# geopti/mjlab-1

Hardware: AMD Instinct MI355X
Metric: env-steps/sec, Unitree-G1 velocity task num_envs=4096, 1/2/4/8 MI355X (higher is better)
Workload: dtype f32

## Files before the change

### mjlab-1_amd/csrc/capi.cpp

```cpp
#include <dlfcn.h>
#include <hip/hip_runtime.h>

#include <cmath>
#include <cstdio>
#include <cstring>
#include <map>
#include <memory>
#include <string>
#include <algorithm>
#include <vector>

#include "../../include/mjx355.h"
#include "engine.h"
#include "model_tables.h"

extern "C" {
typedef struct { int32_t device_type; int32_t device_id; } DLDevice;
typedef struct { uint8_t code; uint8_t bits; uint16_t lanes; } DLDataType;
typedef struct {
  void* data;
  DLDevice device;
  int32_t ndim;
  DLDataType dtype;
  int64_t* shape;
// ... 232 lines not shown
#define X_FLT(name, cnt, w)                                                              \
  {                                                                                      \
    const size_t n_ = (size_t)(cnt) * (w);                                               \
    std::vector<float> h_(desc->name, desc->name + n_);                                  \
    if (upload(m.get(), h_, dm.name)) return -1;                                         \
    dm.name##_ws = 0;                                                                    \
    m->host_float[#name] = std::move(h_);                                                \
    m->float_dims[#name] = {(int64_t)(cnt), (int64_t)(w)};                               \
  }
  MJX_MODEL_INT_FIELDS(X_INT)
  MJX_MODEL_FLOAT_FIELDS(X_FLT)
#undef X_INT
#undef X_FLT
  if (upload(m.get(), std::vector<uint64_t>(desc->dof_bodymask, desc->dof_bodymask + d.nv), dm.dof_bodymask))
    return -1;
  dm.nmaskword = t.nmaskword;
  dm.neq = t.neq;
  dm.max_condim = t.max_condim;
  dm.ncsens = t.ncsens;
  const size_t nmask = (size_t)desc->nmaskword * d.nsensor;
  if (upload(m.get(), t.dof_ancmask, dm.dof_ancmask) || upload(m.get(), t.body_submask, dm.body_submask) ||
      upload(m.get(), t.body_dofmask, dm.body_dofmask) ||
      upload(m.get(), t.body_rec, dm.body_rec, mjx::kBodyRec) ||
      upload(m.get(), t.dof_rec, dm.dof_rec, mjx::kDofRec) ||
      upload(m.get(), t.act_rec, dm.act_rec, mjx::kActRec) ||
      upload(m.get(), t.geom_lds, dm.geom_lds) || upload(m.get(), t.lds_geom, dm.lds_geom) ||
      upload(m.get(), t.st_geom, dm.st_geom) || upload(m.get(), t.st_pairadr, dm.st_pairadr) ||
      upload(m.get(), t.st_partner, dm.st_partner) || upload(m.get(), t.st_aabb, dm.st_aabb, 6) ||
      upload(m.get(), t.st_chunk_aabb, dm.st_chunk_aabb) ||
      (!t.pair_rec.empty() && upload(m.get(), t.pair_rec, dm.pair_rec)) ||
      upload(m.get(), std::vector<uint32_t>(desc->sensor_geommask1, desc->sensor_geommask1 + nmask), dm.sensor_geommask1) ||
      upload(m.get(), std::vector<uint32_t>(desc->sensor_geommask2, desc->sensor_geommask2 + nmask), dm.sensor_geommask2) ||
      upload(m.get(), t.cs_sensor, dm.cs_sensor) || upload(m.get(), t.geom_csmask1, dm.geom_csmask1) ||
      upload(m.get(), t.geom_csmask2, dm.geom_csmask2))
    return -1;
  if (!t.sensor_ext.empty() && upload(m.get(), t.sensor_ext, m->ext.rec)) return -1;
  m->ext.n = (int)t.sensor_ext.size();
  *out = m.release();
  return 0;
}

int mjx_model_destroy(mjxModel* m) {
  if (m) delete m;
  return 0;
}

int mjx_sim_create(const mjxModel* model, int nworld, int nconmax, int njmax, mjxSim** out) {
  return mjx_sim_create_ex(model, nworld, nconmax, njmax, nconmax, njmax, out);
}

int mjx_sim_create_ex(const mjxModel* model, int nworld, int nconmax, int njmax,
                      int nconmax_max, int njmax_max, mjxSim** out) {
  if (!model || !out) return fail("null argument");
  if (nworld <= 0) return fail("nworld must be positive");
  if (nconmax <= 0 || nconmax > mjx::kWave)
    return fail("nconmax (contacts held per world) must be in [1, 64]");
  if (njmax <= 0) return fail("njmax must be positive");
  if (njmax < 2 * model->t.neq)
    return fail("njmax below the model's equality rows (two per equality constraint)");
  if (model->t.max_condim > 3 && njmax_max < 2 * model->t.neq + 2 * (model->t.max_condim - 1))
    return fail("njmax_max below one contact of the model's largest condim (2 (condim - 1) rows "
                "behind the equality rows)");
  if (nconmax_max < nconmax || nconmax_max > mjx::kMaxContacts || njmax_max < njmax)
    return fail("max capacity: nconmax <= nconmax_max <= 512 and njmax <= njmax_max");
  if (nconmax_max > mjx::kWave && nconmax_max > njmax_max)
    return fail("a max capacity past 64 contacts needs njmax_max >= nconmax_max (the contact sort's "
                "scratch is the row block)");
// ... 572 lines not shown
```

### mjlab-1_amd/csrc/engine.h

```cpp
#pragma once

#include <hip/hip_runtime.h>
#include <stddef.h>
#include <stdint.h>

#include "fields.h"

namespace mjx {

constexpr int kWave = 64;
constexpr int kMaxConRounds = 8;
constexpr int kMaxContacts = kWave * kMaxConRounds;
constexpr int kBodyRec = 20, kDofRec = 12, kActRec = 4;
constexpr int kMaxBodies = 64;
constexpr int kMaxDof = 64;
constexpr int kMaxLanes = 64;
constexpr int kRowClasses = 2;
constexpr int kMaxSplit = 4;
constexpr int kSplitMinWorlds = 2048;
constexpr int kMaxAirSlots = 8;
constexpr int kStaticChunk = 64;

enum { EFC_LIMIT = 0, EFC_FRICTIONLESS = 1, EFC_PYRAMIDAL = 2, EFC_EQUALITY = 3 };
constexpr int kMaxEq = 64;
enum { GEOM_PLANE = 0, GEOM_HFIELD = 1, GEOM_SPHERE = 2, GEOM_CAPSULE = 3, GEOM_BOX = 6 };
enum { JNT_FREE = 0, JNT_BALL = 1, JNT_SLIDE = 2, JNT_HINGE = 3 };
enum { SENS_GYRO = 0, SENS_VELOCIMETER = 1, SENS_ACCELEROMETER = 2, SENS_SUBTREEANGMOM = 3,
       SENS_CONTACT = 4, SENS_FRAMEPOS = 5, SENS_FRAMEQUAT = 6, SENS_JOINTPOS = 7,
       SENS_JOINTVEL = 8,
       SENS_FRAMEPOSX = 9, SENS_FRAMEXAXIS = 10, SENS_FRAMEYAXIS = 11, SENS_FRAMEZAXIS = 12,
       SENS_FRAMELINVEL = 13, SENS_FRAMEANGVEL = 14, SENS_FRAMELINACC = 15, SENS_FRAMEANGACC = 16,
       SENS_SUBTREECOM = 17, SENS_SUBTREELINVEL = 18, SENS_ACTUATORPOS = 19, SENS_ACTUATORVEL = 20,
       SENS_ACTUATORFRC = 21, SENS_JOINTACTUATORFRC = 22, SENS_COUNT = 23 };
enum { OBJ_NONE = 0, OBJ_BODY = 1, OBJ_XBODY = 2, OBJ_JOINT = 3, OBJ_GEOM = 5, OBJ_SITE = 6,
       OBJ_ACTUATOR = 19 };
enum { REDUCE_NONE = 0, REDUCE_MINDIST = 1, REDUCE_MAXFORCE = 2, REDUCE_NETFORCE = 3 };

struct Dims {
  int nq, nv, nu, nbody, njnt, ngeom, nsite, nsensor, nsensordata, npair;
  int nhfield, nhfielddata, nlevel, nchild, nmocap;
  int ngeom_lds;
  int npair_all;
  int nstatic;
  int nstpartner;
  int nboxbox;
  int nconmax;
// ... 12 lines not shown
#define X_FLT(name, cnt, w) const float* name; int name##_ws;
  MJX_MODEL_CORE_INT_FIELDS(X_INT)
  MJX_MODEL_CORE_FLOAT_FIELDS(X_FLT)
  const uint64_t* dof_bodymask;
  const uint64_t* dof_ancmask;
  const uint64_t* body_submask;
  const uint64_t* body_dofmask;
  const int32_t* body_rec;
  const int32_t* dof_rec;
  const int32_t* act_rec;
  const int32_t* geom_lds;
  const int32_t* lds_geom;
  const int32_t* st_geom;
  const int32_t* st_pairadr;
  const int32_t* st_partner;
  const float* st_aabb;
  const float* st_chunk_aabb;
  const int32_t* pair_rec;
  int nmaskword;
  const uint32_t* sensor_geommask1;
  const uint32_t* sensor_geommask2;
  int ncsens;
  const int32_t* cs_sensor;
  const uint64_t* geom_csmask1;
  const uint64_t* geom_csmask2;
  MJX_MODEL_EQ_INT_FIELDS(X_INT)
  MJX_MODEL_EQ_FLOAT_FIELDS(X_FLT)
#undef X_INT
#undef X_FLT
  int neq;
  int max_condim;
  int eq_reserved0;
  float* contact_torque;
  int eq_reserved[8];
};
static_assert(sizeof(DModel) - offsetof(DModel, eq_type) == 128, "DModel: the equality block is 128 bytes");

struct DData {
#define X_FLT(name, cnt, w) float* name;
#define X_INT(name, cnt, w) int32_t* name;
  MJX_DATA_FLOAT_FIELDS(X_FLT)
  MJX_DATA_INT_FIELDS(X_INT)
#undef X_FLT
#undef X_INT
  int32_t* stats;
  int32_t* wstats;
  int32_t* evtotal;
  unsigned long long* prof;
  unsigned long long* wtrace;
};

struct Lds {
  int qpos, qvel, ctrl, qacc_ws, qfrc_applied, xfrc;
  int xpos, xquat, xmat, xipos, ximat, xanchor, xaxis;
  int stmass, subtree_com, cinert, crb, cvel, cacc, stlin, stang;
  int cdof, cdofdot, cacc_v, gxpos, gxmat, sxpos, sxmat;
  int M, H;
  int qfrc_bias, qfrc_passive, qfrc_act, qfrc_smooth, qacc_smooth, x, Mx, grad, srch, Ms,
      qfrc_con, vtmp, act_force, act_len, act_vel;
  int con_g1, con_g2, con_key, con_dist, con_pos, con_frame, con_mu, con_kb,
      con_imp, con_imargin, con_dim, con_efc, con_n;
  int efc_J, efc_aref, efc_D, efc_jar, efc_Js, efc_force, efc_cid, efc_act, hdiag;
  int red;
  int chol;
  int ints;
  int pack_len;
  int packC_b;
// ... 169 lines not shown
```

### mjlab-1_amd/csrc/engine_impl.h

```cpp
#pragma once
#include <float.h>
#include <stdlib.h>
#include <algorithm>
#include <initializer_list>
#include <utility>
#include <math.h>

#include "engine.h"

#pragma clang fp contract(on)

namespace mjx {

#define MINVAL 1e-15f
#define MINMU 1e-5f
#define MINIMP 0.0001f
#define MAXIMP 0.9999f


struct V3 { float x, y, z; };
__device__ __forceinline__ V3 v3(const float* p) { return {p[0], p[1], p[2]}; }
__device__ __forceinline__ void st3(float* p, V3 a) { p[0] = a.x; p[1] = a.y; p[2] = a.z; }
__device__ __forceinline__ V3 operator+(V3 a, V3 b) { return {a.x + b.x, a.y + b.y, a.z + b.z}; }
__device__ __forceinline__ V3 operator-(V3 a, V3 b) { return {a.x - b.x, a.y - b.y, a.z - b.z}; }
// ... 506 lines not shown
#pragma unroll
  for (int c = 0; c < NR; c += 4) {
    float4 v = make_float4(0.f, 0.f, 0.f, 0.f);
    if (c < nvp) v = ld4(rp + c);
    A[c] = v.x; A[c + 1] = v.y; A[c + 2] = v.z; A[c + 3] = v.w;
  }
}
template <int NR>
__device__ __forceinline__ void rows_load_factor_ltr(float (&A)[NR], float& rd, const float* Lp,
                                                     int nvp, int lane) {
  const int ln = opaque_lane(lane);
  const int row = ln < nvp ? ln : 0;
  const float* rp = Lp + ltr_off(row);
  rows_load_ltr_span<NR>(A, rp, nvp);
  const float dv = rp[row];
  rd = ln < nvp ? dv : 1.f;
  const float ljj = __builtin_amdgcn_rcpf(rd);
#pragma unroll
  for (int k = 0; k < NR; k++) {
    const float s = rl(rd, k);
    A[k] = k < ln ? A[k] * (s * ljj) : 0.f;
  }
}
template <int NR>
__device__ __forceinline__ void rows_load_factor_ltr_raw(float (&A)[NR], float& dv, const float* Lp,
                                                         int nvp, int lane) {
  const int ln = opaque_lane(lane);
  const int row = ln < nvp ? ln : 0;
  const float* rp = Lp + ltr_off(row);
  const int len = 4 * ((row >> 2) + 1);
#pragma unroll
  for (int c = 0; c < NR; c += 4) {
    const float4 v = ld4(rp + (c < len ? c : 0));
    const bool in = c < len;
    A[c] = in ? v.x : 0.f; A[c + 1] = in ? v.y : 0.f; A[c + 2] = in ? v.z : 0.f; A[c + 3] = in ? v.w : 0.f;
  }
  dv = rp[row];
}
template <int NR>
__device__ __forceinline__ void rows_load_ltr(float (&A)[NR], const float* Lp, int nvp, int lane) {
  rows_load_ltr_span<NR>(A, Lp + ltr_off(lane < nvp ? lane : 0), nvp);
  if (NR > nvp || kWave > NR) {
    const int ln = opaque_lane(lane);
    const bool pad = ln >= nvp;
#pragma unroll
    for (int c = 0; c < NR; c++) A[c] = pad ? (c == ln ? 1.f : 0.f) : A[c];
  }
}
template <int NR>
__device__ __forceinline__ void rows_scale_factor_ltr(float (&A)[NR], float& rd, float dv, int nvp,
                                                      int lane) {
  const int ln = opaque_lane(lane);
  rd = ln < nvp ? dv : 1.f;
  const float ljj = __builtin_amdgcn_rcpf(rd);
#pragma unroll
  for (int k = 0; k < NR; k++) {
    const float s = rl(rd, k);
    A[k] = k < ln ? A[k] * (s * ljj) : 0.f;
  }
}
template <int NR>
__device__ __forceinline__ float rows_solve_ltr(const float (&M)[NR], float rdiag, const float* Lp,
                                                float x, int nvp, int lane) {
  float u = x;
#pragma unroll
  for (int j = 0; j < NR; j++) u = fmaf(-M[j], rl(u, j), u);
  float Nc[NR];
  const int ln = opaque_lane(lane);
  const int col = ln < nvp ? ln : 0;
#pragma unroll
// ... 1014 lines not shown
  unsigned long long z = seed + 0x9E3779B97F4A7C15ull * ((unsigned long long)(unsigned)w + 1) +
                         0xD1B54A32D192ED03ull * (unsigned long long)(unsigned)draw +
                         0x8CB92BA72F3D8DD7ull * (unsigned long long)group;
  z = (z ^ (z >> 30)) * 0xBF58476D1CE4E5B9ull;
  z = (z ^ (z >> 27)) * 0x94D049BB133111EBull;
  return (uint32_t)((z ^ (z >> 31)) >> 32);
}
__device__ __forceinline__ void act_push(const ActParams& A, int w, int u, int nu) {
  if (u >= nu || A.kind[u] == kActBuiltin || A.max_lag[u] == 0) return;
  const int L = A.ring_len;
  const size_t i = (size_t)w * nu + u;
  float* r = A.ring + (size_t)w * L * nu + u;
  for (int k = 0; k + 1 < L; k++) r[(size_t)k * nu] = r[(size_t)(k + 1) * nu];
  r[(size_t)(L - 1) * nu] = A.pt[i];
  A.pushes[i] = min(A.pushes[i] + 1, L);
  const int lo = A.min_lag[u], span = A.max_lag[u] - lo + 1;
  if (span > 1 && !(A.hold && A.hold[i])) {
    const int n = A.draws[i];
    A.lag[i] = lo + (int)(((unsigned long long)act_hash(A.seed, w, A.group[u], n) * (unsigned)span) >> 32);
    A.draws[i] = (int)((unsigned)n + 1u);
  }
}
__device__ __forceinline__ int cb_b1(int v) { return v & 255; }
__device__ __forceinline__ int cb_b2(int v) { return (v >> 8) & 255; }
__device__ __forceinline__ int cb_r1(int v) { return (v >> 16) & 255; }
__device__ __forceinline__ int cb_r2(int v) { return (v >> 24) & 255; }
__device__ __forceinline__ V3 point_vel_r(const float* S, const Lds& L, int b, int root, V3 p) {
  if (b <= 0) return {0.f, 0.f, 0.f};
  const float* cv = S + L.cvel + 6 * b;
  return v3(cv + 3) + cross(v3(cv), p - v3(S + L.subtree_com + 3 * root));
}

__device__ __forceinline__ void contact_sensors_wave(const float* S, const int* Si, const Lds& L,
                                                     const DModel& m, const Dims& d, float* sd,
                                                     int ncon, int maxmatch, bool all,
                                                     const Params* __restrict__ P, int lane,
                                                     int mcd, int cone) {
  const int c = lane;
  const bool valid = c < ncon;
  V3 fg = {0, 0, 0}, fc = {0, 0, 0}, tc = {0, 0, 0};
  float dist = 0.f;
  uint64_t m1 = 0, m2 = 0;
  if (valid) {
    const int g1 = Si[L.con_g1 + c], g2 = Si[L.con_g2 + c];
    m1 = m.geom_csmask1[g1] & m.geom_csmask2[g2];
    m2 = m.geom_csmask1[g2] & m.geom_csmask2[g1];
    if (all) {
      dist = S[L.con_dist + c];
      fc = con_frame_force(S, Si, L, c, mcd, cone);
      fg = frame_tv(S + L.con_n + 3 * c, fc);
      if (mcd > 3) tc = con_frame_torque(S, Si, L, c, cone);
    }
  }
  const int ncs = m.ncsens;
  int dbits = 0, dred = 0, dadr = 0, ddim = 0;
  if (lane < ncs) {
    const int s = m.cs_sensor[lane];
    dbits = m.sensor_intprm[3 * s];
    dred = m.sensor_intprm[3 * s + 1];
    dadr = m.sensor_adr[s];
    ddim = m.sensor_dim[s];
  }
  const bool fonly = lane < ncs && dbits == 1 && ddim == 1;
  const bool mtrunc = maxmatch < ncon;
  const uint64_t below = (1ull << lane) - 1ull;
  const uint64_t mm = m1 | m2;
  float fcount = 0.f;
  uint64_t rest = __ballot(lane < ncs && !fonly);
  for (uint64_t fo = __ballot(fonly); fo; fo &= fo - 1) {
    const int k = __ffsll((long long)fo) - 1;
    const float f = (float)min(__popcll(__ballot((mm >> k) & 1ull)), maxmatch);
    fcount = lane == k ? f : fcount;
  }
  if (fonly) sd[dadr] = fcount;
  for (; rest; rest &= rest - 1) {
    const int k = __ffsll((long long)rest) - 1;
    const int bits = __builtin_amdgcn_readlane(dbits, k), reduce = __builtin_amdgcn_readlane(dred, k);
    const int adr = __builtin_amdgcn_readlane(dadr, k), dim = __builtin_amdgcn_readlane(ddim, k);
    if (!all) {
      bool air = false;
      for (int i = 0; i < P->nair; i++) air |= P->air_found[i] == adr;
      if (!air) continue;
    }
    float* out = sd + adr;
    bool a1 = (m1 >> k) & 1ull, a2 = (m2 >> k) & 1ull;
    if (mtrunc) {
      const bool keep = __popcll(__ballot(a1 || a2) & below) < maxmatch;
      a1 = a1 && keep;
      a2 = a2 && keep;
    }
    const bool match = a1 || a2;
    const unsigned long long bal = __ballot(match);
    const float found = (float)__popcll(bal);
    float v = 0.f;
    if (reduce == REDUCE_NETFORCE) {
      const float sg = match ? (a1 ? 1.f : -1.f) : 0.f;
      const float nx = wave_sum(sg * fg.x), ny = wave_sum(sg * fg.y), nz = wave_sum(sg * fg.z);
      if (bits & 1) v = lane == 0 ? found : 0.f;
      else if (bits & 2) v = lane == 0 ? nx : lane == 1 ? ny : lane == 2 ? nz : 0.f;
    } else {
      int sel = -1;
      if (reduce == REDUCE_NONE) {
        sel = bal ? __ffsll((long long)bal) - 1 : -1;
      } else {
        float key = reduce == REDUCE_MINDIST ? dist : -sqrtf(fc.x * fc.x + fc.y * fc.y + fc.z * fc.z);
        if (!match) key = FLT_MAX;
        const float kmin = wave_min(key);
        const unsigned long long win = __ballot(match && key == kmin);
        sel = win ? __ffsll((long long)win) - 1 : -1;
      }
      if (sel >= 0) {
        const int cs = sel;
        const float sg = rl(a1 ? 1.f : -1.f, cs);
        const int t = lane < 3 ? lane : 0;
        if (bits & 1) v = lane == 0 ? found : 0.f;
        else if (bits & 8) v = lane == 0 ? rl(dist, cs) : 0.f;
        else if (bits & 16) v = lane < 3 ? S[L.con_pos + 3 * cs + t] : 0.f;
        else if (bits & 32) v = lane < 3 ? sg * S[L.con_n + 3 * cs + t] : 0.f;
        else if (bits & 64) v = lane < 3 ? sg * vc(cframe(v3(S + L.con_n + 3 * cs)).t, t) : 0.f;
        else if (bits & 2) {
          const float fx = rl(fc.x, cs), fy = rl(fc.y, cs), fz = rl(fc.z, cs);
          v = lane == 0 ? fx : lane == 1 ? fy : lane == 2 ? fz : 0.f;
        } else if (mcd > 3 && (bits & 4)) {
          const float tx = rl(tc.x, cs), ty = rl(tc.y, cs), tz = rl(tc.z, cs);
          v = lane == 0 ? tx : lane == 1 ? ty : lane == 2 ? tz : 0.f;
        }
      }
    }
    if (lane < dim) out[lane] = v;
  }
}

template <int SP>
constexpr bool lean_spec() {
  if constexpr (SP <= 0) {
    return false;
  } else {
    constexpr Dims d = ModelSpec<SP>::dims();
    return nr_for_nv(d.nv) <= 20 && d.nstatic == 0 && d.nboxbox == 0 &&
           make_lds(d, 0).total * 4 <= 10240 && make_lds(d, 1).total * 4 <= 10240 &&
           make_lds(d, 2).total * 4 <= 10240;
  }
}
template <int SP> constexpr bool kLean = lean_spec<SP>();
enum { kConeTop = 0, kConeQuad = 1, kConeMid = 2 };
__device__ __forceinline__ int cone_zone(float N, float T, float mu) {
  if (!(T > 0.f)) return N >= 0.f ? kConeTop : kConeQuad;
  if (N >= mu * T) return kConeTop;
  if (mu * N + T <= 0.f) return kConeQuad;
  return kConeMid;
}
__device__ __forceinline__ void tiles_add_cone(float (&A)[2][16], const Tiles& T, const float* J,
                                               const int* grp, const float* ca, const float* cc,
                                               const float* dh, const float* wa, const float* wc,
                                               const int* mid, int nmid, int nvp) {
#pragma unroll
  for (int s = 0; s < 2; s++) {
    if (!T.own[s]) continue;
    const int oi = 4 * T.bi[s], oj = 4 * T.bj[s];
    for (int k = 0; k < nmid; k++) {
      const int r0 = mid[k], dim = grp[r0] >> 16;
      float ai[4] = {0, 0, 0, 0}, aj[4] = {0, 0, 0, 0}, ci[4] = {0, 0, 0, 0}, cj[4] = {0, 0, 0, 0};
// ... 2151 lines not shown
      unsigned long long sig_f[4] = {0, 0, 0, 0};
      bool same_f;
      const int nact = reg_rows ? build_active1(act, rja, nefc, lane, sig_f, &same_f)
                                : build_active(act, jar, nefc, lane, sig_f, &same_f);
      sync();
      jt_mul(S + L.qfrc_con, J, wv, act, nact, nvp, lane);
      st.sub(8);
    }
    st.stamp(9);
    if (lane == 0) ints[5] = niter;
    sync();
    cp4(gc + LC.ints, S + L.ints, 8, lane);
    cp4(gc + LC.x, S + L.x, nvq, lane);
    cp4(gc + LC.qfrc_con, S + L.qfrc_con, nvq, lane);
    if (last || P->outputs_every)
      cp4(gc + LC.efc_force, S + L.efc_force, (nefc + 3) & ~3, lane);
    if (last) {
      for (int i = lane; i < nv; i += kWave) {
        size_t k = (size_t)w * nv + i;
        D.qacc[k] = S[L.x + i];
        D.qfrc_constraint[k] = S[L.qfrc_con + i];
      }
      if (lane == 0) D.solver_niter[w] = niter;
    }
    st.stamp(14);
  } else {
    if (last || P->outputs_every) {
      cp_pack(S, gc, L.pack_len, lane);
    } else {
      cp_pack(S, gc, L.packC_sub, lane);
      cp_pack(S + L.ints, gc + L.ints, L.efc_force - L.ints, lane);
    }
    float Fa[NR], Fdv = 1.f;
    if (integrate) rows_load_factor_ltr_raw<NR>(Fa, Fdv, gf, nvp, lane);
    for (int i = lane; i < nvp; i += kWave) {
      const bool in = i < nv;
      S[L.qvel + i] = in ? D.qvel[(size_t)w * nv + i] : 0.f;
      S[L.qacc_ws + i] = in ? D.qacc_warmstart[(size_t)w * nv + i] : 0.f;
    }
    for (int i = lane; i < nq; i += kWave) S[L.qpos + i] = D.qpos[(size_t)w * nq + i];
    float time = D.time[w];
    const BodyLite B = load_body_lite(m, d, min(lane, nb - 1));
    const bool bl = lane < nb;
    lds_dma_wait();
    sync();
    const int nefc = ints[1];
    int ncon = ints[4];
    const int niter_last = ints[5];
    st.stamp(15);
    if (last || P->outputs_every) {
      float a[6];
#pragma unroll
      for (int t = 0; t < 6; t++) a[t] = S[L.cacc_v + 6 * B.b + t];
#pragma unroll 4
      for (int j = 0; j < nv; j++) {
        const float fa = (B.dofs >> j) & 1ull ? S[L.x + j] : 0.f;
        const float* cd = S + L.cdof + 6 * j;
#pragma unroll
        for (int t = 0; t < 6; t += 2) {
          const float2 c2 = *reinterpret_cast<const float2*>(cd + t);
          a[t] = fmaf(fa, c2.x, a[t]);
          a[t + 1] = fmaf(fa, c2.y, a[t + 1]);
        }
      }
      if (bl) {
#pragma unroll
        for (int t = 0; t < 6; t++) S[L.cacc + 6 * B.b + t] = a[t];
      }
    }
    sync();
    st.stamp(10);
    for (int s = lane; s < d.nsensor; s += kWave) {
      float* out = D.sensordata + (size_t)w * d.nsensordata + m.sensor_adr[s];
      int obj = m.sensor_objid[s];
      int type = m.sensor_type[s];
      if ((type == SENS_ACCELEROMETER || type == SENS_CONTACT) != (PH == 2)) continue;
      if (!last && !P->outputs_every) {
        if (type != SENS_CONTACT) continue;
        bool air = false;
        for (int i = 0; i < P->nair; i++) air |= P->air_found[i] == m.sensor_adr[s];
        if (!air) continue;
      }
      if (type == SENS_CONTACT && m.sensor_intprm[3 * s + 2] <= 1 && m.ncsens > 0 &&
          (kCon1<SP> || ncon <= kWave)) continue;
      if (type == SENS_GYRO || type == SENS_VELOCIMETER || type == SENS_ACCELEROMETER) {
        int b = m.site_bodyid[obj];
        const float* R = S + L.sxmat + 9 * obj;
        const float* cv = S + L.cvel + 6 * b;
        V3 rel = v3(S + L.sxpos + 3 * obj) - v3(S + L.subtree_com + 3 * m.body_rootid[b]);
        V3 r;
        if (type == SENS_GYRO) {
          r = mulTv(R, v3(cv));
        } else {
          V3 v = v3(cv + 3) + cross(v3(cv), rel);
          if (type == SENS_VELOCIMETER) {
            r = mulTv(R, v);
          } else {
            const float* ca = S + L.cacc + 6 * b;
            V3 a = v3(ca + 3) + cross(v3(ca), rel) + cross(v3(cv), v);
            r = mulTv(R, a);
          }
        }
        out[0] = r.x; out[1] = r.y; out[2] = r.z;
      } else if (type == SENS_SUBTREEANGMOM) {
      } else if (type == SENS_FRAMEPOS) {
        const float* p = m.sensor_objtype[s] == OBJ_SITE ? S + L.sxpos + 3 * obj : S + L.xpos + 3 * obj;
        out[0] = p[0]; out[1] = p[1]; out[2] = p[2];
      } else if (type == SENS_JOINTPOS) {
        out[0] = S[L.qpos + m.jnt_qposadr[obj]];
      } else if (type == SENS_JOINTVEL) {
        out[0] = S[L.qvel + m.jnt_dofadr[obj]];
      } else if (type == SENS_CONTACT) {
        const int32_t* ip = m.sensor_intprm + 3 * s;
        int bits = ip[0], reduce = ip[1], nslot = min(ip[2], 8);
        const uint32_t* mk1 = m.sensor_geommask1 + m.nmaskword * s;
        const uint32_t* mk2 = m.sensor_geommask2 + m.nmaskword * s;
        int fdim = ((bits & 1) || (bits & 8)) ? 1 : 3;
        int dim = m.sensor_dim[s];
        for (int i = 0; i < dim; i++) out[i] = 0.f;
        int found = 0;
        V3 net = {0, 0, 0};
        int sel[8];
        float key[8];
        int nsel = 0;
        for (int c = 0; c < ncon; c++) {
          int g1 = Si[L.con_g1 + c], g2 = Si[L.con_g2 + c];
          bool a1 = ((mk1[g1 >> 5] >> (g1 & 31)) & 1u) && ((mk2[g2 >> 5] >> (g2 & 31)) & 1u);
          bool a2 = ((mk1[g2 >> 5] >> (g2 & 31)) & 1u) && ((mk2[g1 >> 5] >> (g1 & 31)) & 1u);
          if (!a1 && !a2) continue;
          if (found >= o.maxmatch) continue;
          found++;
          const V3 f = con_frame_force(S, Si, L, c, mcd, cone);
          V3 fg = frame_tv(S + L.con_n + 3 * c, f);
          net = net + fg * (a1 ? 1.f : -1.f);
          float k = reduce == REDUCE_MINDIST ? S[L.con_dist + c]
                  : reduce == REDUCE_MAXFORCE ? -norm(f) : (float)nsel;
          if (nsel < nslot || k < key[nsel - 1]) {
            int pos = nsel < nslot ? nsel++ : nslot - 1;
            while (pos > 0 && key[pos - 1] > k) { key[pos] = key[pos - 1]; sel[pos] = sel[pos - 1]; pos--; }
            key[pos] = k;
            sel[pos] = c * 2 + (a1 ? 0 : 1);
          }
        }
        if (reduce == REDUCE_NETFORCE) {
          if (bits & 1) out[0] = (float)found;
          else if (bits & 2) { out[0] = net.x; out[1] = net.y; out[2] = net.z; }
        } else {
          for (int k = 0; k < nsel; k++) {
            int c = sel[k] >> 1;
            float sg = (sel[k] & 1) ? -1.f : 1.f;
            float* oo = out + k * fdim;
            if (bits & 1) oo[0] = (float)found;
            else if (bits & 8) oo[0] = S[L.con_dist + c];
            else if (bits & 16) { for (int t = 0; t < 3; t++) oo[t] = S[L.con_pos + 3 * c + t]; }
            else if (bits & 32) { for (int t = 0; t < 3; t++) oo[t] = sg * S[L.con_n + 3 * c + t]; }
            else if (bits & 64) { for (int t = 0; t < 3; t++) oo[t] = sg * vc(cframe(v3(S + L.con_n + 3 * c)).t, t); }
            else if (bits & 2) {
              const V3 f = con_frame_force(S, Si, L, c, mcd, cone);
              oo[0] = f.x; oo[1] = f.y; oo[2] = f.z;
            } else if (mcd > 3 && (bits & 4)) {
              const V3 t = con_frame_torque(S, Si, L, c, cone);
              oo[0] = t.x; oo[1] = t.y; oo[2] = t.z;
            }
          }
        }
      }
    }
    if (kCon1<SP> || ncon <= kWave)
      contact_sensors_wave(S, Si, L, m, d, D.sensordata + (size_t)w * d.nsensordata, ncon,
                           o.maxmatch, last || P->outputs_every, P, lane, mcd, cone);
    st.stamp(11);
    if (last) {
      size_t wb = (size_t)w * nb;
      for (int i = lane; i < 6 * nb; i += kWave) D.cacc[wb * 6 + i] = S[L.cacc + i];
      size_t wc = (size_t)w * P->con_stride;
      const int nout = min(P->con_stride, D.wstats[8 * (size_t)w + 6]);
      for (int c = lane; c < nout; c += kWave) {
        V3 f = {0, 0, 0};
        if (c < ncon && nefc > 0) f = con_frame_force(S, Si, L, c, mcd, cone);
        D.contact_force[(wc + c) * 3] = f.x;
        D.contact_force[(wc + c) * 3 + 1] = f.y;
        D.contact_force[(wc + c) * 3 + 2] = f.z;
        if (mcd > 3) {
          V3 t = {0, 0, 0};
          if (c < ncon && nefc > 0) t = con_frame_torque(S, Si, L, c, cone);
          float* ct = m.contact_torque + (wc + c) * 3;
          ct[0] = t.x; ct[1] = t.y; ct[2] = t.z;
        }
      }
    }
    if (lane < 6) {
      int* ws = D.wstats + 8 * (size_t)w;
      const int v = lane == 0 ? ints[0] : lane == 1 ? nefc : lane == 5 ? niter_last
                  : (ints[3] >> (lane - 2)) & 1;
      const int old = ws[lane];
      ws[lane] = (lane >= 2 && lane <= 4) ? old + v : max(old, v);
      if (lane >= 2 && lane <= 4 && v) atomicAdd(D.evtotal + lane - 2, v);
    }
    st.stamp(12);
    st.sub_restart();
    if (integrate) {
      sync();
    sync();
    {
      st.sub(9);
      st.sub(10);
      {
        float rd;
        rows_scale_factor_ltr<NR>(Fa, rd, Fdv, nvp, lane);
        const int pl = kTree<SP> ? nvp - 1 - lane : lane;
        const float f = lane < nvp ? S[L.qfrc_smooth + pl] + S[L.qfrc_con + pl] : 0.f;
        const float acc = rows_solve_ltr<NR>(Fa, rd, gf, f, nvp, lane);
        if (lane < nvp && pl < nv) S[L.qvel + pl] += h * acc;
      }
      sync();
      st.sub(11);
      for (int k = lane; k < d.njnt; k += kWave) {
        int a = m.jnt_qposadr[k], dof = m.jnt_dofadr[k];
        int t = m.jnt_type[k];
        if (t == JNT_FREE) {
          for (int i = 0; i < 3; i++) S[L.qpos + a + i] += h * S[L.qvel + dof + i];
          V3 wv = v3(S + L.qvel + dof + 3);
          float nw = norm(wv);
          V3 ax = nw < MINVAL ? V3{1, 0, 0} : wv * (1.0f / nw);
          Q4 q = qnorm(q4(S + L.qpos + a + 3));
          q = qmul(q, qaxisangle(ax, h * nw));
          st4(S + L.qpos + a + 3, q);
        } else if (t == JNT_HINGE || t == JNT_SLIDE) {
          S[L.qpos + a] += h * S[L.qvel + dof];
        }
      }
      for (int i = lane; i < nv; i += kWave) S[L.qacc_ws + i] = S[L.x + i];
      time += h;
      sync();
      st.sub(12);
    }

      for (int i = lane; i < nq; i += kWave) D.qpos[(size_t)w * nq + i] = S[L.qpos + i];
      for (int i = lane; i < nv; i += kWave) {
        D.qvel[(size_t)w * nv + i] = S[L.qvel + i];
        D.qacc_warmstart[(size_t)w * nv + i] = S[L.qacc_ws + i];
      }
      if (lane == 0) D.time[w] = time;
      const int nair = P->nair;
      if (nair > 0) {
        __builtin_amdgcn_fence(__ATOMIC_RELEASE, "workgroup");
        __builtin_amdgcn_fence(__ATOMIC_ACQUIRE, "workgroup");
        const float el = time - P->air_time[w];
        if (lane < nair) {
          const size_t i = (size_t)w * nair + lane;
          const bool contact = D.sensordata[(size_t)w * d.nsensordata + P->air_found[lane]] > 0.f;
          const float ca = P->air_cur[i], cc = P->air_cc[i];
          if (ca > 0.f && contact) P->air_last[i] = ca + el;
          P->air_cur[i] = contact ? 0.f : ca + el;
          if (cc > 0.f && !contact) P->air_lc[i] = cc + el;
          P->air_cc[i] = contact ? cc + el : 0.f;
        }
        if (lane == 0) P->air_time[w] = time;
      }
      if (P->act_on && P->act.ring_len > 0) act_push(P->act, w, lane, nu);
      if constexpr (NETC) {
        if (P->act_on && P->net.hist_len > 0) net_push(P->net, w, lane, nu);
      }
    }
    st.stamp(13);
  }
  st.flush(P, PH, w, lane);
}

__device__ __forceinline__ bool ovf_more(const Params* __restrict__ P, int sel, int bid) {
  if (!(sel & kSelOvf)) return false;
  const int li = 2 * (sel & 0xff) + ((sel & kSelRPar) ? 1 : 0);
  if (bid >= min(P->ovf_n[li], P->ovf_cap)) return false;
  __syncthreads();
  return true;
}

template <int NR, int PH, int SP, int NET = 0>
__global__ __launch_bounds__(kWave) MJX_PHASE_ATTR void step_phase(const Params* __restrict__ P, int w0, int w1,
                                                    int sel, int last, int integrate,
                                                    const uint8_t* __restrict__ mask) {
  extern __shared__ __attribute__((aligned(16))) float S[];
  step_body<NR, PH, SP, NET ? 4 : 0>(S, P, w0, w1, sel, last, PH == 1 ? 0 : integrate,
                                     PH == 1 ? integrate : 0, mask, (int)blockIdx.x);
}
template <int NR, int SP, int JGL = 1, int CAP = 0>
__global__ __launch_bounds__(kWave) __attribute__((amdgpu_waves_per_eu(CAP ? 3 : 1, CAP ? 8 : 2))) void step_newton_lat(
    const Params* __restrict__ P, int w0, int w1, int sel, int last, int row_class,
    const uint8_t* __restrict__ mask) {
  extern __shared__ __attribute__((aligned(16))) float S[];
  step_body<NR, 1, SP, JGL>(S, P, w0, w1, sel, last, 0, row_class, mask, (int)blockIdx.x);
}
template <int NR, int SP>
__global__ __launch_bounds__(kWave) MJX_PHASE_ATTR_B void step_phase_jg(
    const Params* __restrict__ P, int w0, int w1, int sel, int last, int row_class,
// ... 158 lines not shown
```

### mjlab-1_amd/csrc/model_tables.h

```cpp
#pragma once

#include <algorithm>
#include <cmath>
#include <cstring>
#include <string>
#include <vector>

#include "../../include/mjx355.h"
#include "engine.h"

namespace mjx {

struct ModelTables {
  Dims d{};
  Opt o{};
  int nmaskword = 0;
  int neq = 0;
  int max_condim = 3;
  int ncsens = 0;
  std::vector<int32_t> dof_parentid;
  std::vector<uint64_t> dof_ancmask, body_submask, body_dofmask;
  std::vector<int32_t> body_rec, dof_rec, act_rec;
  std::vector<int32_t> geom_lds, lds_geom;
  std::vector<int32_t> st_geom, st_pairadr, st_partner;
  std::vector<float> st_aabb, st_chunk_aabb;
  std::vector<int32_t> pair_rec;
  std::vector<int32_t> cs_sensor;
  std::vector<uint64_t> geom_csmask1, geom_csmask2;
  std::vector<int32_t> static_geoms;
  std::vector<float> static_xpos, static_xmat;
  std::vector<SensorExtRec> sensor_ext;
};

namespace tables {

inline bool is_static(const mjxModelDesc& desc, int g) {
  const int t = desc.geom_type[g];
  return t == GEOM_HFIELD || (t == GEOM_BOX && desc.body_weldid[desc.geom_bodyid[g]] == 0);
}

inline std::string check_limits(const mjxModelDesc& desc) {
  if (desc.abi_version != MJX_ABI_VERSION) return "ABI version mismatch";
  if (desc.nbody > kMaxBodies) return "at most 64 bodies per world supported";
  if (desc.nv > kMaxDof) return "at most 64 dofs per world supported";
  if (desc.nv > 60)
    return "at most 60 dofs per world supported (61 to 64 need a third register tile per lane)";
  if (desc.nbody > 0 && desc.level_body && desc.body_rootid) {
    auto is_free = [&](int b) {
      return desc.body_jntnum[b] > 0 && desc.jnt_type[desc.body_jntadr[b]] == 0;
    };
    for (int b = 1; b < desc.nbody; b++) {
      const int r = desc.body_rootid[b];
      if (r < 0 || r >= desc.nbody) return "body_rootid out of range";
      const int x = desc.level_body[r];
      if (x != r && (is_free(r) || is_free(x)))
        return "a tree that follows a tree of several bodies is not supported: its root's "
               "body id is not its level-order lane (one articulated tree, then single bodies)";
    }
  }
  if (desc.nu > kMaxLanes || desc.njnt > kMaxLanes)
    return "at most 64 actuators and 64 joints per world supported";
// ... 294 lines not shown
  if (!packable) return;
  std::vector<int32_t>& rec = t.pair_rec;
  rec.resize((size_t)4 * nreg);
  for (int q = 0; q < nreg; q++) {
    const int g1 = desc.pair_geom1[q], g2 = desc.pair_geom2[q];
    const int t1 = desc.geom_type[g1], t2 = desc.geom_type[g2];
    const float r1 = (float)desc.geom_rbound[g1], r2 = (float)desc.geom_rbound[g2];
    const float mg = std::fmax((float)desc.geom_margin[g1], (float)desc.geom_margin[g2]);
    const float cull = (r1 > 0 && r2 > 0 && t1 != GEOM_HFIELD) ? r1 + r2 + mg : INFINITY;
    rec[4 * q] = g1 | g2 << 16;
    rec[4 * q + 1] = t.geom_lds[g1] | t.geom_lds[g2] << 12 | t1 << 24 | (int32_t)((uint32_t)t2 << 28);
    std::memcpy(&rec[4 * q + 2], &mg, 4);
    std::memcpy(&rec[4 * q + 3], &cull, 4);
  }
}

inline void contact_sensor_masks(const mjxModelDesc& desc, ModelTables& t) {
  std::vector<int32_t>& cs = t.cs_sensor;
  for (int s = 0; s < desc.nsensor; s++)
    if (desc.sensor_type[s] == SENS_CONTACT && desc.sensor_intprm[3 * s + 2] <= 1) cs.push_back(s);
  t.geom_csmask1.assign(desc.ngeom, 0);
  t.geom_csmask2.assign(desc.ngeom, 0);
  t.ncsens = cs.size() <= 64 ? (int)cs.size() : 0;
  for (int k = 0; k < t.ncsens; k++) {
    const uint32_t* a = desc.sensor_geommask1 + (size_t)desc.nmaskword * cs[k];
    const uint32_t* b = desc.sensor_geommask2 + (size_t)desc.nmaskword * cs[k];
    for (int g = 0; g < desc.ngeom; g++) {
      if ((a[g >> 5] >> (g & 31)) & 1u) t.geom_csmask1[g] |= 1ull << k;
      if ((b[g >> 5] >> (g & 31)) & 1u) t.geom_csmask2[g] |= 1ull << k;
    }
  }
}

}

inline std::string build_model_tables(const mjxModelDesc& desc, ModelTables& t) {
  std::string err = tables::check_limits(desc);
  if (err.empty()) err = tables::check_equalities(desc);
  if (err.empty()) err = tables::check_condims(desc, t.max_condim);
  if (err.empty()) err = tables::build_sensor_ext(desc, t.sensor_ext);
  if (err.empty() && desc.nmaskword < (desc.ngeom + 31) / 32) err = "nmaskword < ceil(ngeom / 32)";
  if (!err.empty()) return err;
  t.nmaskword = desc.nmaskword;
  tables::dims_and_options(desc, t);
  tables::tree_tables(desc, t);
  err = tables::terrain_blocks(desc, t);
  if (err.empty()) err = tables::terrain_frames(desc, t);
  if (!err.empty()) return err;
  tables::pair_records(desc, t);
  tables::contact_sensor_masks(desc, t);
  return "";
}

}
```

Before: 3.090 million.

## Pack sensor and joint records and prefetch phase-C inputs before the LDS DMA wait

Builds packed per-sensor, per-contact-sensor and per-joint int records on the host, and loads them as vector loads. They are prefetched, together with qvel, qpos, warmstart, wstats and air-time state, into registers before the LDS DMA wait, so that latency overlaps the DMA. The velocity solve is moved ahead of the sensor stage. Air-time contact values are captured from registers during the contact-sensor pass, which avoids a fence and a global re-read of sensordata. In exchange it adds register pressure, loads the factor unconditionally, and drops the non-accelerometer sensor branches, which assumes this phase only handles accelerometer and contact sensors.

```diff
diff --git a/mjlab-1_amd/csrc/capi.cpp b/mjlab-1_amd/csrc/capi.cpp
--- a/mjlab-1_amd/csrc/capi.cpp
+++ b/mjlab-1_amd/csrc/capi.cpp
@@ -288,7 +288,10 @@
       upload(m.get(), std::vector<uint32_t>(desc->sensor_geommask1, desc->sensor_geommask1 + nmask), dm.sensor_geommask1) ||
       upload(m.get(), std::vector<uint32_t>(desc->sensor_geommask2, desc->sensor_geommask2 + nmask), dm.sensor_geommask2) ||
       upload(m.get(), t.cs_sensor, dm.cs_sensor) || upload(m.get(), t.geom_csmask1, dm.geom_csmask1) ||
-      upload(m.get(), t.geom_csmask2, dm.geom_csmask2))
+      upload(m.get(), t.geom_csmask2, dm.geom_csmask2) ||
+      upload(m.get(), t.sens_rec, dm.sens_rec, mjx::kSensRec) ||
+      upload(m.get(), t.cs_rec, dm.cs_rec, mjx::kCsRec) ||
+      upload(m.get(), t.jnt_rec, dm.jnt_rec, mjx::kJntRec))
     return -1;
   if (!t.sensor_ext.empty() && upload(m.get(), t.sensor_ext, m->ext.rec)) return -1;
   m->ext.n = (int)t.sensor_ext.size();
diff --git a/mjlab-1_amd/csrc/engine.h b/mjlab-1_amd/csrc/engine.h
--- a/mjlab-1_amd/csrc/engine.h
+++ b/mjlab-1_amd/csrc/engine.h
@@ -12,6 +12,7 @@
 constexpr int kMaxConRounds = 8;
 constexpr int kMaxContacts = kWave * kMaxConRounds;
 constexpr int kBodyRec = 20, kDofRec = 12, kActRec = 4;
+constexpr int kSensRec = 12, kCsRec = 4, kJntRec = 4;
 constexpr int kMaxBodies = 64;
 constexpr int kMaxDof = 64;
 constexpr int kMaxLanes = 64;
@@ -90,7 +91,10 @@
   int max_condim;
   int eq_reserved0;
   float* contact_torque;
-  int eq_reserved[8];
+  const int32_t* sens_rec;
+  const int32_t* cs_rec;
+  const int32_t* jnt_rec;
+  int eq_reserved[2];
 };
 static_assert(sizeof(DModel) - offsetof(DModel, eq_type) == 128, "DModel: the equality block is 128 bytes");
 
diff --git a/mjlab-1_amd/csrc/engine_impl.h b/mjlab-1_amd/csrc/engine_impl.h
--- a/mjlab-1_amd/csrc/engine_impl.h
+++ b/mjlab-1_amd/csrc/engine_impl.h
@@ -562,10 +562,17 @@
 #pragma unroll
   for (int c = 0; c < NR; c += 4) {
     const float4 v = ld4(rp + (c < len ? c : 0));
-    const bool in = c < len;
-    A[c] = in ? v.x : 0.f; A[c + 1] = in ? v.y : 0.f; A[c + 2] = in ? v.z : 0.f; A[c + 3] = in ? v.w : 0.f;
+    A[c] = v.x; A[c + 1] = v.y; A[c + 2] = v.z; A[c + 3] = v.w;
   }
   dv = rp[row];
+}
+template <int NR>
+__device__ __forceinline__ void rows_mask_factor_ltr_raw(float (&A)[NR], int nvp, int lane) {
+  const int ln = opaque_lane(lane);
+  const int row = ln < nvp ? ln : 0;
+  const int len = 4 * ((row >> 2) + 1);
+#pragma unroll
+  for (int c = 0; c < NR; c++) A[c] = c < len ? A[c] : 0.f;
 }
 template <int NR>
 __device__ __forceinline__ void rows_load_ltr(float (&A)[NR], const float* Lp, int nvp, int lane) {
@@ -1646,35 +1653,22 @@
 }
 
 __device__ __forceinline__ void contact_sensors_wave(const float* S, const int* Si, const Lds& L,
-                                                     const DModel& m, const Dims& d, float* sd,
-                                                     int ncon, int maxmatch, bool all,
-                                                     const Params* __restrict__ P, int lane,
-                                                     int mcd, int cone) {
+                                                     float* sd, int ncon, int ncs, int maxmatch,
+                                                     bool all, uint64_t m1, uint64_t m2, int4 csr,
+                                                     const int (&af)[kMaxAirSlots], int nair,
+                                                     int air_adr, float& air_val, bool& air_got,
+                                                     int lane, int mcd, int cone) {
   const int c = lane;
   const bool valid = c < ncon;
   V3 fg = {0, 0, 0}, fc = {0, 0, 0}, tc = {0, 0, 0};
   float dist = 0.f;
-  uint64_t m1 = 0, m2 = 0;
-  if (valid) {
-    const int g1 = Si[L.con_g1 + c], g2 = Si[L.con_g2 + c];
-    m1 = m.geom_csmask1[g1] & m.geom_csmask2[g2];
-    m2 = m.geom_csmask1[g2] & m.geom_csmask2[g1];
-    if (all) {
-      dist = S[L.con_dist + c];
-      fc = con_frame_force(S, Si, L, c, mcd, cone);
-      fg = frame_tv(S + L.con_n + 3 * c, fc);
-      if (mcd > 3) tc = con_frame_torque(S, Si, L, c, cone);
-    }
-  }
-  const int ncs = m.ncsens;
-  int dbits = 0, dred = 0, dadr = 0, ddim = 0;
-  if (lane < ncs) {
-    const int s = m.cs_sensor[lane];
-    dbits = m.sensor_intprm[3 * s];
-    dred = m.sensor_intprm[3 * s + 1];
-    dadr = m.sensor_adr[s];
-    ddim = m.sensor_dim[s];
-  }
+  if (valid && all) {
+    dist = S[L.con_dist + c];
+    fc = con_frame_force(S, Si, L, c, mcd, cone);
+    fg = frame_tv(S + L.con_n + 3 * c, fc);
+    if (mcd > 3) tc = con_frame_torque(S, Si, L, c, cone);
+  }
+  const int dbits = csr.x, dred = csr.y, dadr = csr.z, ddim = csr.w;
   const bool fonly = lane < ncs && dbits == 1 && ddim == 1;
   const bool mtrunc = maxmatch < ncon;
   const uint64_t below = (1ull << lane) - 1ull;
@@ -1687,13 +1681,23 @@
     fcount = lane == k ? f : fcount;
   }
   if (fonly) sd[dadr] = fcount;
+  if (nair > 0) {
+#pragma unroll
+    for (int i = 0; i < kMaxAirSlots; i++) {
+      const unsigned long long hit = __ballot(fonly && dadr == af[i]);
+      if (!hit) continue;
+      const float f = rl(fcount, __ffsll((long long)hit) - 1);
+      if (lane == i) { air_val = f; air_got = true; }
+    }
+  }
   for (; rest; rest &= rest - 1) {
     const int k = __ffsll((long long)rest) - 1;
     const int bits = __builtin_amdgcn_readlane(dbits, k), reduce = __builtin_amdgcn_readlane(dred, k);
     const int adr = __builtin_amdgcn_readlane(dadr, k), dim = __builtin_amdgcn_readlane(ddim, k);
     if (!all) {
       bool air = false;
-      for (int i = 0; i < P->nair; i++) air |= P->air_found[i] == adr;
+#pragma unroll
+      for (int i = 0; i < kMaxAirSlots; i++) air |= af[i] == adr;
       if (!air) continue;
     }
     float* out = sd + adr;
@@ -1742,6 +1746,12 @@
       }
     }
     if (lane < dim) out[lane] = v;
+    const int off = air_adr - adr;
+    const bool mine = off >= 0 && off < dim;
+    if (__ballot(mine)) {
+      const float t = __shfl(v, mine ? off : 0);
+      if (mine) { air_val = t; air_got = true; }
+    }
   }
 }
 
@@ -3959,23 +3969,76 @@
       cp_pack(S + L.ints, gc + L.ints, L.efc_force - L.ints, lane);
     }
     float Fa[NR], Fdv = 1.f;
-    if (integrate) rows_load_factor_ltr_raw<NR>(Fa, Fdv, gf, nvp, lane);
-    for (int i = lane; i < nvp; i += kWave) {
-      const bool in = i < nv;
-      S[L.qvel + i] = in ? D.qvel[(size_t)w * nv + i] : 0.f;
-      S[L.qacc_ws + i] = in ? D.qacc_warmstart[(size_t)w * nv + i] : 0.f;
-    }
-    for (int i = lane; i < nq; i += kWave) S[L.qpos + i] = D.qpos[(size_t)w * nq + i];
-    float time = D.time[w];
+    rows_load_factor_ltr_raw<NR>(Fa, Fdv, gf, nvp, lane);
+    const float* const dflt = D.time + w;
+    float r_qvel = *(lane < nv ? D.qvel + (size_t)w * nv + lane : dflt);
+    float r_qaw = *(lane < nv ? D.qacc_warmstart + (size_t)w * nv + lane : dflt);
+    const float r_qpos = *(lane < nq ? D.qpos + (size_t)w * nq + lane : dflt);
+    float time = *dflt;
     const BodyLite B = load_body_lite(m, d, min(lane, nb - 1));
     const bool bl = lane < nb;
+    const int nair = P->nair, con_stride = P->con_stride;
+    const bool all_out = last || P->outputs_every;
+    const bool ring_on = (P->act_on != 0) & (P->act.ring_len > 0);
+    bool hist_on = false;
+    if constexpr (NETC) hist_on = (P->act_on != 0) & (P->net.hist_len > 0);
+    const int ncs = m.ncsens;
+    const int4* srec = reinterpret_cast<const int4*>(m.sens_rec + (size_t)kSensRec * (lane < d.nsensor ? lane : 0));
+    int4 sr0 = srec[0], sr1 = srec[1];
+    int2 sr2 = *reinterpret_cast<const int2*>(srec + 2);
+    int4 csr = *reinterpret_cast<const int4*>(m.cs_rec + (size_t)kCsRec * (lane < ncs ? lane : 0));
+    int4 jr = *reinterpret_cast<const int4*>(m.jnt_rec + (size_t)kJntRec * (lane < d.njnt ? lane : 0));
+    int* ws = D.wstats + 8 * (size_t)w;
+    int ws_old = ws[lane & 7];
+    int air_adr = P->air_found[lane & (kMaxAirSlots - 1)];
+    const bool air_on = integrate && nair > 0;
+    const size_t ai = (size_t)w * nair + (lane < nair ? lane : 0);
+    const float *acur = P->air_cur, *accn = P->air_cc, *atime = P->air_time;
+    asm volatile("" : "+v"(acur), "+v"(accn), "+v"(atime));
+    float air_ca = *(air_on ? acur + ai : dflt);
+    float air_c = *(air_on ? accn + ai : dflt);
+    const float air_t0 = *(air_on ? atime + w : dflt);
     lds_dma_wait();
+    asm volatile("" : "+v"(sr0.x), "+v"(sr0.y), "+v"(sr0.z), "+v"(sr0.w), "+v"(sr1.x), "+v"(sr1.y),
+                 "+v"(sr1.z), "+v"(sr1.w), "+v"(sr2.x), "+v"(sr2.y));
+    asm volatile("" : "+v"(csr.x), "+v"(csr.y), "+v"(csr.z), "+v"(csr.w), "+v"(jr.x), "+v"(jr.y),
+                 "+v"(jr.z), "+v"(ws_old), "+v"(air_adr), "+v"(air_ca), "+v"(air_c));
+    asm volatile("" : "+v"(r_qvel), "+v"(r_qaw));
+    rows_mask_factor_ltr_raw<NR>(Fa, nvp, lane);
+    air_adr = lane < nair ? air_adr : -1;
+    if (lane < nvp) {
+      S[L.qvel + lane] = lane < nv ? r_qvel : 0.f;
+      S[L.qacc_ws + lane] = lane < nv ? r_qaw : 0.f;
+    }
+    if (lane < nq) S[L.qpos + lane] = r_qpos;
+    for (int i = lane + kWave; i < nq; i += kWave) S[L.qpos + i] = D.qpos[(size_t)w * nq + i];
     sync();
     const int nefc = ints[1];
     int ncon = ints[4];
     const int niter_last = ints[5];
     st.stamp(15);
-    if (last || P->outputs_every) {
+    const bool cwave = kCon1<SP> || ncon <= kWave;
+    uint64_t cm1 = 0, cm2 = 0, cm3 = 0, cm4 = 0;
+    if (cwave && ncs > 0 && lane < ncon) {
+      const int g1 = Si[L.con_g1 + lane], g2 = Si[L.con_g2 + lane];
+      cm1 = m.geom_csmask1[g1]; cm2 = m.geom_csmask2[g2];
+      cm3 = m.geom_csmask1[g2]; cm4 = m.geom_csmask2[g1];
+    }
+    float acc = 0.f;
+    if (integrate) {
+      float rd;
+      rows_scale_factor_ltr<NR>(Fa, rd, Fdv, nvp, lane);
+      const int pl = kTree<SP> ? nvp - 1 - lane : lane;
+      const float f = lane < nvp ? S[L.qfrc_smooth + pl] + S[L.qfrc_con + pl] : 0.f;
+      acc = rows_solve_ltr<NR>(Fa, rd, gf, f, nvp, lane);
+    }
+    int af[kMaxAirSlots];
+#pragma unroll
+    for (int i = 0; i < kMaxAirSlots; i++)
+      af[i] = i < nair ? __builtin_amdgcn_readlane(air_adr, i) : -1;
+    float air_val = 0.f;
+    bool air_got = false;
+    if (all_out) {
       float a[6];
 #pragma unroll
       for (int t = 0; t < 6; t++) a[t] = S[L.cacc_v + 6 * B.b + t];
@@ -3997,53 +4060,40 @@
     }
     sync();
     st.stamp(10);
+    float* const sd = D.sensordata + (size_t)w * d.nsensordata;
     for (int s = lane; s < d.nsensor; s += kWave) {
-      float* out = D.sensordata + (size_t)w * d.nsensordata + m.sensor_adr[s];
-      int obj = m.sensor_objid[s];
-      int type = m.sensor_type[s];
-      if ((type == SENS_ACCELEROMETER || type == SENS_CONTACT) != (PH == 2)) continue;
-      if (!last && !P->outputs_every) {
+      if (s >= kWave) {
+        const int4* rec = reinterpret_cast<const int4*>(m.sens_rec + (size_t)kSensRec * s);
+        sr0 = rec[0]; sr1 = rec[1];
+        sr2 = *reinterpret_cast<const int2*>(rec + 2);
+      }
+      const int type = sr0.x, obj = sr0.z;
+      float* out = sd + sr0.w;
+      if (type != SENS_ACCELEROMETER && type != SENS_CONTACT) continue;
+      if (!all_out) {
         if (type != SENS_CONTACT) continue;
         bool air = false;
-        for (int i = 0; i < P->nair; i++) air |= P->air_found[i] == m.sensor_adr[s];
+#pragma unroll
+        for (int i = 0; i < kMaxAirSlots; i++) air |= af[i] == sr0.w;
         if (!air) continue;
       }
-      if (type == SENS_CONTACT && m.sensor_intprm[3 * s + 2] <= 1 && m.ncsens > 0 &&
-          (kCon1<SP> || ncon <= kWave)) continue;
-      if (type == SENS_GYRO || type == SENS_VELOCIMETER || type == SENS_ACCELEROMETER) {
-        int b = m.site_bodyid[obj];
+      if (type == SENS_CONTACT && sr1.w <= 1 && ncs > 0 && cwave) continue;
+      if (type == SENS_ACCELEROMETER) {
+        const int b = sr2.x;
         const float* R = S + L.sxmat + 9 * obj;
         const float* cv = S + L.cvel + 6 * b;
-        V3 rel = v3(S + L.sxpos + 3 * obj) - v3(S + L.subtree_com + 3 * m.body_rootid[b]);
-        V3 r;
-        if (type == SENS_GYRO) {
-          r = mulTv(R, v3(cv));
-        } else {
-          V3 v = v3(cv + 3) + cross(v3(cv), rel);
-          if (type == SENS_VELOCIMETER) {
-            r = mulTv(R, v);
-          } else {
-            const float* ca = S + L.cacc + 6 * b;
-            V3 a = v3(ca + 3) + cross(v3(ca), rel) + cross(v3(cv), v);
-            r = mulTv(R, a);
-          }
-        }
+        V3 rel = v3(S + L.sxpos + 3 * obj) - v3(S + L.subtree_com + 3 * sr2.y);
+        V3 v = v3(cv + 3) + cross(v3(cv), rel);
+        const float* ca = S + L.cacc + 6 * b;
+        V3 a = v3(ca + 3) + cross(v3(ca), rel) + cross(v3(cv), v);
+        V3 r = mulTv(R, a);
         out[0] = r.x; out[1] = r.y; out[2] = r.z;
-      } else if (type == SENS_SUBTREEANGMOM) {
-      } else if (type == SENS_FRAMEPOS) {
-        const float* p = m.sensor_objtype[s] == OBJ_SITE ? S + L.sxpos + 3 * obj : S + L.xpos + 3 * obj;
-        out[0] = p[0]; out[1] = p[1]; out[2] = p[2];
-      } else if (type == SENS_JOINTPOS) {
-        out[0] = S[L.qpos + m.jnt_qposadr[obj]];
-      } else if (type == SENS_JOINTVEL) {
-        out[0] = S[L.qvel + m.jnt_dofadr[obj]];
-      } else if (type == SENS_CONTACT) {
-        const int32_t* ip = m.sensor_intprm + 3 * s;
-        int bits = ip[0], reduce = ip[1], nslot = min(ip[2], 8);
+      } else {
+        int bits = sr1.y, reduce = sr1.z, nslot = min(sr1.w, 8);
         const uint32_t* mk1 = m.sensor_geommask1 + m.nmaskword * s;
         const uint32_t* mk2 = m.sensor_geommask2 + m.nmaskword * s;
         int fdim = ((bits & 1) || (bits & 8)) ? 1 : 3;
-        int dim = m.sensor_dim[s];
+        int dim = sr1.x;
         for (int i = 0; i < dim; i++) out[i] = 0.f;
         int found = 0;
         V3 net = {0, 0, 0};
@@ -4093,15 +4143,15 @@
         }
       }
     }
-    if (kCon1<SP> || ncon <= kWave)
-      contact_sensors_wave(S, Si, L, m, d, D.sensordata + (size_t)w * d.nsensordata, ncon,
-                           o.maxmatch, last || P->outputs_every, P, lane, mcd, cone);
+    if (cwave)
+      contact_sensors_wave(S, Si, L, sd, ncon, ncs, o.maxmatch, all_out, cm1 & cm2, cm3 & cm4, csr,
+                           af, nair, air_adr, air_val, air_got, lane, mcd, cone);
     st.stamp(11);
     if (last) {
       size_t wb = (size_t)w * nb;
       for (int i = lane; i < 6 * nb; i += kWave) D.cacc[wb * 6 + i] = S[L.cacc + i];
-      size_t wc = (size_t)w * P->con_stride;
-      const int nout = min(P->con_stride, D.wstats[8 * (size_t)w + 6]);
+      size_t wc = (size_t)w * con_stride;
+      const int nout = min(con_stride, __builtin_amdgcn_readlane(ws_old, 6));
       for (int c = lane; c < nout; c += kWave) {
         V3 f = {0, 0, 0};
         if (c < ncon && nefc > 0) f = con_frame_force(S, Si, L, c, mcd, cone);
@@ -4117,10 +4167,9 @@
       }
     }
     if (lane < 6) {
-      int* ws = D.wstats + 8 * (size_t)w;
       const int v = lane == 0 ? ints[0] : lane == 1 ? nefc : lane == 5 ? niter_last
                   : (ints[3] >> (lane - 2)) & 1;
-      const int old = ws[lane];
+      const int old = ws_old;
       ws[lane] = (lane >= 2 && lane <= 4) ? old + v : max(old, v);
       if (lane >= 2 && lane <= 4 && v) atomicAdd(D.evtotal + lane - 2, v);
     }
@@ -4133,18 +4182,13 @@
       st.sub(9);
       st.sub(10);
       {
-        float rd;
-        rows_scale_factor_ltr<NR>(Fa, rd, Fdv, nvp, lane);
         const int pl = kTree<SP> ? nvp - 1 - lane : lane;
-        const float f = lane < nvp ? S[L.qfrc_smooth + pl] + S[L.qfrc_con + pl] : 0.f;
-        const float acc = rows_solve_ltr<NR>(Fa, rd, gf, f, nvp, lane);
         if (lane < nvp && pl < nv) S[L.qvel + pl] += h * acc;
       }
       sync();
       st.sub(11);
-      for (int k = lane; k < d.njnt; k += kWave) {
-        int a = m.jnt_qposadr[k], dof = m.jnt_dofadr[k];
-        int t = m.jnt_type[k];
+      if (lane < d.njnt) {
+        const int a = jr.x, dof = jr.y, t = jr.z;
         if (t == JNT_FREE) {
           for (int i = 0; i < 3; i++) S[L.qpos + a + i] += h * S[L.qvel + dof + i];
           V3 wv = v3(S + L.qvel + dof + 3);
@@ -4169,15 +4213,18 @@
         D.qacc_warmstart[(size_t)w * nv + i] = S[L.qacc_ws + i];
       }
       if (lane == 0) D.time[w] = time;
-      const int nair = P->nair;
       if (nair > 0) {
-        __builtin_amdgcn_fence(__ATOMIC_RELEASE, "workgroup");
-        __builtin_amdgcn_fence(__ATOMIC_ACQUIRE, "workgroup");
-        const float el = time - P->air_time[w];
-        if (lane < nair) {
+        const bool slot = lane < nair;
+        if (__ballot(slot && !air_got)) {
+          __builtin_amdgcn_fence(__ATOMIC_RELEASE, "workgroup");
+          __builtin_amdgcn_fence(__ATOMIC_ACQUIRE, "workgroup");
+          if (slot && !air_got) air_val = sd[air_adr];
+        }
+        const float el = time - air_t0;
+        if (slot) {
           const size_t i = (size_t)w * nair + lane;
-          const bool contact = D.sensordata[(size_t)w * d.nsensordata + P->air_found[lane]] > 0.f;
-          const float ca = P->air_cur[i], cc = P->air_cc[i];
+          const bool contact = air_val > 0.f;
+          const float ca = air_ca, cc = air_c;
           if (ca > 0.f && contact) P->air_last[i] = ca + el;
           P->air_cur[i] = contact ? 0.f : ca + el;
           if (cc > 0.f && !contact) P->air_lc[i] = cc + el;
@@ -4185,9 +4232,9 @@
         }
         if (lane == 0) P->air_time[w] = time;
       }
-      if (P->act_on && P->act.ring_len > 0) act_push(P->act, w, lane, nu);
+      if (ring_on) act_push(P->act, w, lane, nu);
       if constexpr (NETC) {
-        if (P->act_on && P->net.hist_len > 0) net_push(P->net, w, lane, nu);
+        if (hist_on) net_push(P->net, w, lane, nu);
       }
     }
     st.stamp(13);
diff --git a/mjlab-1_amd/csrc/model_tables.h b/mjlab-1_amd/csrc/model_tables.h
--- a/mjlab-1_amd/csrc/model_tables.h
+++ b/mjlab-1_amd/csrc/model_tables.h
@@ -27,6 +27,7 @@
   std::vector<int32_t> pair_rec;
   std::vector<int32_t> cs_sensor;
   std::vector<uint64_t> geom_csmask1, geom_csmask2;
+  std::vector<int32_t> sens_rec, cs_rec, jnt_rec;
   std::vector<int32_t> static_geoms;
   std::vector<float> static_xpos, static_xmat;
   std::vector<SensorExtRec> sensor_ext;
@@ -387,6 +388,37 @@
   }
 }
 
+inline void phase_c_records(const mjxModelDesc& desc, ModelTables& t) {
+  const int ns = desc.nsensor, nj = desc.njnt;
+  t.sens_rec.assign((size_t)kSensRec * ns, 0);
+  for (int s = 0; s < ns; s++) {
+    int32_t* r = t.sens_rec.data() + (size_t)kSensRec * s;
+    const int type = desc.sensor_type[s], ot = desc.sensor_objtype[s], oi = desc.sensor_objid[s];
+    r[0] = type; r[1] = ot; r[2] = oi; r[3] = desc.sensor_adr[s];
+    r[4] = desc.sensor_dim[s];
+    for (int c = 0; c < 3; c++) r[5 + c] = desc.sensor_intprm[3 * s + c];
+    const bool site = ot == OBJ_SITE || type == SENS_GYRO || type == SENS_VELOCIMETER ||
+                      type == SENS_ACCELEROMETER;
+    int body = -1;
+    if (site) body = oi >= 0 && oi < desc.nsite ? desc.site_bodyid[oi] : -1;
+    else if (ot == OBJ_BODY || ot == OBJ_XBODY) body = oi;
+    if (body >= 0 && body < desc.nbody) { r[8] = body; r[9] = desc.body_rootid[body]; }
+  }
+  const int ncs = (int)t.cs_sensor.size();
+  t.cs_rec.assign((size_t)kCsRec * ncs, 0);
+  for (int k = 0; k < ncs; k++) {
+    const int s = t.cs_sensor[k];
+    int32_t* r = t.cs_rec.data() + (size_t)kCsRec * k;
+    r[0] = desc.sensor_intprm[3 * s]; r[1] = desc.sensor_intprm[3 * s + 1];
+    r[2] = desc.sensor_adr[s]; r[3] = desc.sensor_dim[s];
+  }
+  t.jnt_rec.assign((size_t)kJntRec * nj, 0);
+  for (int j = 0; j < nj; j++) {
+    int32_t* r = t.jnt_rec.data() + (size_t)kJntRec * j;
+    r[0] = desc.jnt_qposadr[j]; r[1] = desc.jnt_dofadr[j]; r[2] = desc.jnt_type[j];
+  }
+}
+
 }
 
 inline std::string build_model_tables(const mjxModelDesc& desc, ModelTables& t) {
@@ -404,7 +436,8 @@
   if (!err.empty()) return err;
   tables::pair_records(desc, t);
   tables::contact_sensor_masks(desc, t);
-  return "";
-}
-
-}
+  tables::phase_c_records(desc, t);
+  return "";
+}
+
+}
```

New measurement: 3.113 million, median of 6. No clear change (+0.7%).
